# gergely-flamich/compression-without-quantization

Measured on AMD Instinct MI355X. Metric: latent blocks encoded/s at KL=16 bits, higher is better.
Workload: dtype f32

## Files before the change

### compression_without_quantization_amd/csrc/cwq_kernels.hip

```cpp
#include <hip/hip_runtime.h>

#include <type_traits>
#include <stdint.h>

#include "cwq_device.h"
#include "cwq_kernels.h"
#include "cwq_refill.h"
#include "cwq_tau_guess.h"

namespace cwq {

__global__ void __launch_bounds__(256) k_prep_dims(
    const float* __restrict__ t_scale, const float* __restrict__ p_loc,
    const float* __restrict__ p_scale, int64_t n, float nst, float sdiv, float rho,
    float* __restrict__ loc_s, float* __restrict__ scale_s, float* __restrict__ lognorm,
    float* __restrict__ out_sample, unsigned long long* __restrict__ keys, int64_t nb) {
  for (int64_t g = blockIdx.x * (int64_t)blockDim.x + threadIdx.x; g < nb;
       g += (int64_t)gridDim.x * blockDim.x)
    keys[g] = 0ull;
  for (int64_t i = blockIdx.x * (int64_t)blockDim.x + threadIdx.x; i < n;
       i += (int64_t)gridDim.x * blockDim.x) {
    float ls, ss;
    shard_consts(p_loc[i], p_scale[i], nst, sdiv, rho, ls, ss);
    loc_s[i] = ls;
    scale_s[i] = ss;
    lognorm[i] = lognorm_of(t_scale[i]);
    out_sample[i] = 0.0f;
  }
}

template <int DC, bool STEP0>
__device__ __forceinline__ float eval_row(const PhiloxStream& st, uint64_t kbase, int64_t d_rt,
                                          int align_rt, const float* __restrict__ loc_s,
                                          const float* __restrict__ scale_s,
                                          const float* __restrict__ mu,
                                          const float* __restrict__ sg,
                                          const float* __restrict__ lognorm,
                                          const float* __restrict__ best,
                                          const double* logtab) {
  return eval_row_f<DC>(st, kbase, d_rt, align_rt, logtab, [&](int64_t e, float zz) -> float {
    float s = scale_s[e] * zz;
    s = loc_s[e] + s;
    const float tv = STEP0 ? s : best[e] + s;
    return log_prob(tv, mu[e], sg[e], lognorm[e]);
  });
}

template <int DC, bool STEP0>
__global__ void __launch_bounds__(256) k_encode_eval(
    const float* __restrict__ t_loc, const float* __restrict__ t_scale,
    const float* __restrict__ loc_s, const float* __restrict__ scale_s,
    const float* __restrict__ lognorm, const float* __restrict__ best,
    const int64_t* __restrict__ block_off, int64_t ud, int64_t ntiles, int64_t tiles_per_block,
    int64_t cand_per_tile, int64_t n_cand, SeedSpec sd, int32_t step,
    unsigned long long* __restrict__ keys) {
  __shared__ double logtab[32];
  __shared__ unsigned long long wkey[4];
  fill_logtab(logtab);
  const uint32_t wv = wave_id();
  const uint32_t lane = threadIdx.x & 63u;

  for (int64_t tile = blockIdx.x; tile < ntiles; tile += gridDim.x) {
    const int64_t g = tile / tiles_per_block;
    const int64_t tt = tile - g * tiles_per_block;
    const BlockSpan sp = block_span(block_off, ud, g);
    const int64_t n0 = tt * cand_per_tile;
    const int64_t n1 = (n0 + cand_per_tile < n_cand) ? n0 + cand_per_tile : n_cand;
    const PhiloxStream st =
        generate_key(step_seed(sd.of(g), step), 42);
    const int align = (int)(((uint64_t)(n0 + wv) * (uint64_t)sp.d) & 3u);

    uint64_t bestk = 0;
    for (int64_t n = n0 + 4 * (int64_t)lane + wv; n < n1; n += 256) {
      const float v = eval_row<DC, STEP0>(st, (uint64_t)n * (uint64_t)sp.d, sp.d, align,
                                          loc_s + sp.off, scale_s + sp.off, t_loc + sp.off,
                                          t_scale + sp.off, lognorm + sp.off,
                                          STEP0 ? nullptr : best + sp.off, logtab);
      const uint64_t k = argmax_key(v, (uint32_t)n);
      bestk = k > bestk ? k : bestk;
    }
    bestk = wave_max_u64(bestk);
    if (lane == 0) wkey[wv] = bestk;
    __syncthreads();
    if (threadIdx.x == 0) {
      uint64_t m = wkey[0];
      for (int i = 1; i < 4; ++i) m = wkey[i] > m ? wkey[i] : m;
      if (m) atomicMax(&keys[g], (unsigned long long)m);
    }
    __syncthreads();
  }
}

constexpr float kPruneC1 = 0x1p-14f;
#ifndef CWQ_PRUNE_MIN_WAVES
#define CWQ_PRUNE_MIN_WAVES 6
#endif
#ifndef CWQ_XCD_BALANCE
#define CWQ_XCD_BALANCE 1
#endif
#ifndef CWQ_TAU_SHARE_MASK
#define CWQ_TAU_SHARE_MASK 7u
#endif
#ifndef CWQ_CSR_TAU_SHARE_MASK
#define CWQ_CSR_TAU_SHARE_MASK 15u
#endif
#ifndef CWQ_SURVIVOR_CAP
#define CWQ_SURVIVOR_CAP 1024
#endif
#ifndef CWQ_LINKED_VISIT
#define CWQ_LINKED_VISIT 1
#endif
#ifndef CWQ_FOLD_ROUND0
#define CWQ_FOLD_ROUND0 1
#endif
#ifndef CWQ_BORROW_REFILL
#define CWQ_BORROW_REFILL 1
#endif
#ifndef CWQ_POOL_RANGE_SKIP
#define CWQ_POOL_RANGE_SKIP 1
#endif
#ifndef CWQ_PARK_COMPLETE
#define CWQ_PARK_COMPLETE 1
#endif
#ifndef CWQ_PARK_MIN_ROWS
#define CWQ_PARK_MIN_ROWS 8192
#endif
#ifndef CWQ_PARK_MIN_D
#define CWQ_PARK_MIN_D 16
#endif
#if CWQ_PARK_COMPLETE && !(CWQ_LINKED_VISIT && CWQ_BORROW_REFILL)
#error "CWQ_PARK_COMPLETE needs CWQ_LINKED_VISIT and CWQ_BORROW_REFILL"
#endif

template <bool STEP0>
__device__ __forceinline__ float cand_diff(float z, float ls, float ss, float mu, float bb) {
  const float s = shard_sample(ls, ss, z);
  const float tv = STEP0 ? s : bb + s;
  return tv - mu;
}
__device__ __forceinline__ float lp_from_z(float z, float cc) {
  const float u = -0.5f * (z * z);
  return u - cc;
}


struct VisitRec {
  float4 sa, sb;
  uint32_t add[2];
  int bk;
  int next;
};
static_assert(sizeof(VisitRec) == 48, "VisitRec: 48 bytes");

template <int D, bool STEP0>
__device__ __forceinline__ float score_rows_wave(
    const PhiloxStream& st, const uint32_t* rows, uint32_t cnt, const float* __restrict__ loc_s,
    const float* __restrict__ scale_s, const float* __restrict__ mu,
    const float* __restrict__ sg, const float* __restrict__ lognorm,
    const float* __restrict__ best, const double* logtab, float* buf, uint32_t lane) {
  constexpr uint32_t G = D / 4;
  const uint32_t r = lane / G, u = lane - r * G;
  if (r < cnt) {
    const F4 z = normal4_dev(st, (uint64_t)rows[r] * G + u, logtab);
#pragma unroll
    for (int t = 0; t < 4; ++t) {
      const uint32_t j = 4u * u + (uint32_t)t;
      const float zz = t == 0 ? z.a : (t == 1 ? z.b : (t == 2 ? z.c : z.d));
      float v = scale_s[j] * zz;
      v = loc_s[j] + v;
      const float tv = STEP0 ? v : best[j] + v;
      buf[r * D + j] = log_prob(tv, mu[j], sg[j], lognorm[j]);
    }
  }
  __builtin_amdgcn_fence(__ATOMIC_SEQ_CST, "wavefront");
  __builtin_amdgcn_wave_barrier();
  float acc = 0.0f;
  const uint32_t fr = lane >> 3;
  if (fr < cnt)
    for (uint32_t e = lane & 7u; e < (uint32_t)D; e += 8u) acc = acc + buf[fr * D + e];
  __builtin_amdgcn_fence(__ATOMIC_SEQ_CST, "wavefront");
  __builtin_amdgcn_wave_barrier();
  float p[8];
#pragma unroll
  for (int l = 0; l < 8; ++l) p[l] = __shfl(acc, (int)((lane & ~7u) + (uint32_t)l), 64);
  return eigen_fold8(p, 0.0f);
}

#ifdef CWQ_TILE_TIMES
constexpr int kTileTimes = 1 << 18;
__device__ unsigned long long g_tile_t0[kTileTimes], g_tile_t1[kTileTimes];
__device__ unsigned int g_tile_wg[kTileTimes];
#endif
#ifdef CWQ_PRUNE_STATS
__device__ unsigned long long g_prune_stats[72];
constexpr int kDbgBlocks = 1 << 20;
__device__ unsigned long long g_dbg_best[kDbgBlocks];
__device__ int g_seed_tau;
#endif

struct TauGuessWaveDims {
  float w, b2;
  int d;
  __device__ __forceinline__ int count() const { return d; }
  template <class F>
  __device__ __forceinline__ cwq::TauGuessSums sum(F f) const {
    cwq::TauGuessSums o = f(w, b2);
#pragma unroll
    for (int sh = 32; sh >= 1; sh >>= 1) {
      o.k += __shfl_xor(o.k, sh, 64);
      o.k1 += __shfl_xor(o.k1, sh, 64);
      o.k2 += __shfl_xor(o.k2, sh, 64);
    }
    return o;
  }
};
__device__ __forceinline__ uint64_t sgpr_pair_uniform(uint64_t v) {
  const uint32_t lo = (uint32_t)__builtin_amdgcn_readfirstlane((int)(uint32_t)v);
  const uint32_t hi = (uint32_t)__builtin_amdgcn_readfirstlane((int)(uint32_t)(v >> 32));
  return ((uint64_t)hi << 32) | lo;
}
constexpr float kTauForceRetry = -2.0f;
__device__ __forceinline__ float tau_guess_of(float qm, float As, float Pq) {
  if (qm == kTauForceRetry) return 3.402823466e+38f;
  if (!(qm >= 0.0f)) return -__builtin_inff();
  const float tg = cwq::screen_row_lower(-qm, cwq::kScreenC2, As, Pq);
  return tg == tg ? tg : -__builtin_inff();
}

template <int D, bool STEP0, bool INTER, bool PARK>
__global__ void __launch_bounds__(256, CWQ_PRUNE_MIN_WAVES) k_encode_prune(
    const float* __restrict__ t_loc, const float* __restrict__ t_scale,
    const float* __restrict__ loc_s, const float* __restrict__ scale_s,
    const float* __restrict__ lognorm, const float* __restrict__ best, int64_t ntiles,
    int64_t tiles_per_block, int64_t cand_per_tile, int64_t n_cand, SeedSpec sd, int32_t step,
    int allow_screen, unsigned long long* __restrict__ keys, int64_t tail_from, int tail_div,
    uint32_t* __restrict__ tq) {
  static_assert(D % 8 == 0 && D >= 8 && D <= 64, "pruned path: D % 8 == 0, D <= 64");
  static_assert(!PARK || CWQ_PARK_COMPLETE, "PARK instances exist in CWQ_PARK_COMPLETE builds only");
  constexpr int G = D / 4;
  constexpr int NF = STEP0 ? 6 : 7;
  constexpr int RW = (64 / G) < 8 ? (64 / G) : 8;
  __shared__ double logtab[32];
  __shared__ float4 cst[G * NF];
  constexpr int NREC = CWQ_FOLD_ROUND0 ? 4 : 1;
  constexpr int RPW = G + (PARK ? 1 : 0);
  __shared__ VisitRec vrec[NREC * RPW];
  __shared__ uint32_t w0g_cell[4];
  __shared__ int2 meta[G];
  __shared__ float rowbuf[4][RW * D];
  __shared__ float dscore[D];
  __shared__ float dA[D];
  __shared__ float dC[D];
  __shared__ float gscore[G];
  __shared__ int gpos[G];
  __shared__ float lowc;
  __shared__ float scr_a, scr_pq;
  __shared__ float tau_cell;
  __shared__ float tau_seed_cell;
  __shared__ float qm_cell;
  __shared__ uint32_t sq_cnt;
  __shared__ uint32_t sq_n[CWQ_SURVIVOR_CAP];
  __shared__ float sq_ub[CWQ_SURVIVOR_CAP];
  __shared__ unsigned long long wkey[4];
  __shared__ uint32_t s_next;
#ifdef CWQ_PRUNE_STATS
  __shared__ uint32_t s_ps[72];
  for (int i = threadIdx.x; i < 72; i += blockDim.x) s_ps[i] = 0u;
#endif
  fill_logtab(logtab);
  const uint32_t wv = wave_id();
  const uint32_t lane = threadIdx.x & 63u;

  constexpr bool inter = INTER;
  const int64_t nbt = INTER ? ntiles / tiles_per_block : 0;
  auto next_tile = [&](int64_t cur) -> int64_t {
    if (tq == nullptr) return cur + gridDim.x;
    __syncthreads();
    if (threadIdx.x == 0) s_next = gridDim.x + atomicAdd(tq, 1u);
    __syncthreads();
    return (int64_t)s_next;
  };
  for (int64_t tile = blockIdx.x; tile < ntiles; tile = next_tile(tile)) {
    uint32_t tid = threadIdx.x;
    asm volatile("" : "+v"(tid));
#ifdef CWQ_TILE_TIMES
    if (tid == 0 && tile < kTileTimes) {
      g_tile_t0[tile] = __builtin_amdgcn_s_memrealtime();
      const uint32_t xcc = (uint32_t)__builtin_amdgcn_s_getreg((20) | (0 << 6) | ((4 - 1) << 11));
      g_tile_wg[tile] = (xcc << 24) | (blockIdx.x & 0xffffffu);
    }
#endif
    int64_t tord = tile;
    const int64_t treg = inter ? nbt * tail_from : 0;
    if (inter && CWQ_XCD_BALANCE && tq == nullptr && tile < treg && (treg & 7) == 0 &&
        (gridDim.x & 7u) == 0)
      tord = (tile & 7) * (treg >> 3) + (tile >> 3);
    const int64_t g = inter ? tord % nbt : tile / tiles_per_block;
    const int64_t tt = inter ? tord / nbt : tile - g * tiles_per_block;
    const int64_t off = g * D;
    int64_t n0, csz;
    if (tt < tail_from) {
      n0 = tt * cand_per_tile;
      csz = cand_per_tile;
    } else {
      csz = cand_per_tile / tail_div;
      n0 = tail_from * cand_per_tile + (tt - tail_from) * csz;
    }
    const int64_t n1 = (n0 + csz < n_cand) ? n0 + csz : n_cand;
    if (n0 >= n1) continue;
    const PhiloxStream st =
        generate_key(step_seed(sd.of(g), step), 42);

    if (tid < D) {
      const int j = tid;
      const float ls = loc_s[off + j], ss = scale_s[off + j], mu = t_loc[off + j];
      const float rs = 1.0f / t_scale[off + j];
      const float m = (STEP0 ? ls : best[off + j] + ls) - mu;
      float e = 0.5f * (ss * ss + m * m) * (rs * rs);
      dscore[j] = (e == e) ? e : -1.0f;
    }
    __syncthreads();
    if (tid < G) {
      const int q = tid;
      gscore[q] = ((dscore[4 * q] + dscore[4 * q + 1]) + dscore[4 * q + 2]) + dscore[4 * q + 3];
    }
    __syncthreads();
    if (tid < G) {
      const int q = tid;
      const float sq = gscore[q];
      int r = 0;
      for (int q2 = 0; q2 < G; ++q2) {
        const float s2 = gscore[q2];
        r += (s2 > sq || (s2 == sq && q2 < q)) ? 1 : 0;
      }
      gpos[q] = r;
      meta[r].x = q;
#pragma unroll
      for (int w = 0; w < NREC; ++w) {
        const uint32_t wg = (uint32_t)(n0 + (int64_t)w * ((n1 - n0 + 3) / 4)) * (uint32_t)G;
        const uint64_t add =
            CWQ_FOLD_ROUND0 ? cwq::philox_round0_addend(wg + (uint32_t)q) : (uint64_t)q;
        VisitRec& v = vrec[w * RPW + r];
        v.add[0] = (uint32_t)add;
        v.add[1] = (uint32_t)(add >> 32);
        v.next = (r + 1 < G || PARK) ? (w * RPW + r + 1) * (int)sizeof(VisitRec) : 0;
      }
    }
    if (PARK && tid >= 64 && tid < 64 + NREC) {
      VisitRec& v = vrec[(tid - 64) * RPW + G];
      v.sa = float4{0.f, 0.f, 0.f, 0.f};
      v.sb = float4{0.f, 0.f, 0.f, 0.f};
      v.add[0] = 0u;
      v.add[1] = 0u;
      v.bk = (int)f2u(__builtin_inff());
      v.next = (int)((tid - 64) * RPW + G) * (int)sizeof(VisitRec);
    }
    __syncthreads();
    int den_ok = 1, scr_ok = 1;
    if (tid < D) {
      const int j = tid, k = gpos[j >> 2], w = j & 3;
      float fj[7];
      const float sgj = t_scale[off + j];
      fj[0] = loc_s[off + j];
      fj[1] = scale_s[off + j];
      fj[2] = t_loc[off + j];
      fj[3] = sgj;
      fj[4] = lognorm[off + j];
      fj[5] = 1.0f / sgj;
      fj[6] = STEP0 ? 0.0f : best[off + j];
      float* c = reinterpret_cast<float*>(cst);
#pragma unroll
      for (int f = 0; f < NF; ++f) c[(k * NF + f) * 4 + w] = fj[f];
      den_ok = markstein_ok_den(sgj) ? 1 : 0;
      const ScreenDim o = screen_dim<STEP0>(fj[0], fj[1], fj[2], sgj, fj[4], fj[6]);
#pragma unroll
      for (int c = 0; c < NREC; ++c) {
        float* sc = reinterpret_cast<float*>(&vrec[c * RPW + k]);
        sc[w] = o.sa;
        sc[4 + w] = o.sb;
      }
      dA[j] = o.A;
      dC[j] = o.C;
      scr_ok = o.ok ? 1 : 0;
    }
    const bool fastdiv = __syncthreads_and(den_ok) != 0;
    const bool scr_all = __syncthreads_and(scr_ok) != 0;
    const bool screen = (allow_screen & 1) && scr_all;
    if (wv == 1u) {
      const int gmode = (allow_screen >> 1) & 3;
      float qm = cwq::kTauNoGuess;
      if (screen && gmode == 1) {
        float w = 0.0f, b2 = 0.0f;
        if (lane < (uint32_t)D) {
          const float* sc = reinterpret_cast<const float*>(&vrec[lane >> 2]);
          const float al = sc[lane & 3u] * (float)(1.0 / cwq::kSqrt2Ln2);
          const float be = sc[4u + (lane & 3u)];
          w = al * al;
          b2 = be * be;
        }
        qm = cwq::tau_guess_q(TauGuessWaveDims{w, b2, D}, n1 - n0, cwq::kTauGuessM);
      } else if (screen && gmode == 2) {
        qm = kTauForceRetry;
      }
      if (lane == 0) qm_cell = qm;
    }
    if (tid <= G + 1) {
      const int kb = tid;
      const float* c = reinterpret_cast<const float*>(cst);
      double rf = 0.0, kk = 0.0, asum = 0.0, msum = 0.0, kall = 0.0, cvis = 0.0, a2 = 0.0,
             amax = 0.0;
#pragma unroll 1
      for (int p = 0; p < D; ++p) {
        const double mj = -(double)c[((p >> 2) * NF + 4) * 4 + (p & 3)];
        const double aj = __builtin_fabs(mj);
        asum += aj;
        msum += mj;
        kall += aj + mj;
        if (p >= 4 * kb) {
          rf += mj + 0x1p-17 * aj;
        } else {
          kk += aj + mj;
          if (screen) cvis += (double)dC[(meta[p >> 2].x << 2) + (p & 3)];
        }
        if (screen && kb == G + 1) {
          const double av = (double)dA[p];
          a2 += av * av;
          amax = av > amax ? av : amax;
        }
      }
      const double marg = 0x1p-20 * (__builtin_fabs(rf) + asum) + 0x1p-126;
      const double sl = 0x1p-14 * (__builtin_fabs(msum) + asum + kall) + 0x1p-126;
      if (kb <= G) {
        const float bk = screen ? round_up_f32(msum + cvis * (1.0 + 0x1p-20) + sl)
                                : round_up_f32(rf + 0x1p-14 * kk + marg);
        if (kb >= 1) {
          meta[kb - 1].y = (int)f2u(bk);
#pragma unroll
          for (int c = 0; c < NREC; ++c) vrec[c * RPW + kb - 1].bk = (int)f2u(bk);
        }
        if (kb == G) lowc = round_up_f32(0x1p-14 * kk + marg);
      } else if (screen) {
        scr_a = screen_as(msum, sl, a2);
        scr_pq = screen_pq(amax, D);
      }
      if (kb == 0) {
        float t0 = -__builtin_inff();
        if (inter) {
          const unsigned long long kv =
              __hip_atomic_load(&keys[g], __ATOMIC_RELAXED, __HIP_MEMORY_SCOPE_AGENT);
          if ((uint32_t)(kv >> 32) > kArgmaxClampOrd) t0 = unord_f32((uint32_t)(kv >> 32));
        }
#ifdef CWQ_PRUNE_STATS
        if (g_seed_tau && g < kDbgBlocks && (g_dbg_best[g] >> 32) > kArgmaxClampOrd)
          t0 = unord_f32((uint32_t)(g_dbg_best[g] >> 32));
#endif
        tau_cell = t0;
        tau_seed_cell = t0;
        sq_cnt = 0u;
      }
    }
    __syncthreads();
    const float lc = lowc;
#ifdef CWQ_PRUNE_STATS
    const float tau_seed = tau_cell;
#endif
    const float sA = scr_a, sPq = scr_pq;

    const int64_t per_wave = (n1 - n0 + 3) / 4;
    const int64_t w0 = n0 + (int64_t)wv * per_wave;
    const int64_t w1 = (w0 + per_wave < n1) ? w0 + per_wave : n1;
    const uint32_t w0g =
        (uint32_t)__builtin_amdgcn_readfirstlane((int)((uint32_t)w0 * (uint32_t)G));
    if (lane == 0) w0g_cell[wv] = w0g;
    const uint32_t wrows = w1 > w0 ? (uint32_t)(w1 - w0) : 0u;
    const uint32_t ng_end =
        (uint32_t)__builtin_amdgcn_readfirstlane((int)(wrows * (uint32_t)G));
    const uint32_t ng_stat = (uint32_t)__builtin_amdgcn_readfirstlane(
        (int)(cwq::refill_static_rows(wrows) * (uint32_t)G));
    const uint32_t ng_pool0 = (uint32_t)__builtin_amdgcn_readfirstlane(
        (int)(cwq::refill_pool_start(cwq::refill_static_rows(wrows)) * (uint32_t)G));
    const uint32_t ng_first =
        (CWQ_BORROW_REFILL && ng_stat != 0u) ? ng_stat - 64u * (uint32_t)G : 0u;
    const uint32_t kbase = CWQ_FOLD_ROUND0 ? wv * (uint32_t)(RPW * sizeof(VisitRec)) : 0u;
#ifndef CWQ_TAU_FROM_KEYS
#define CWQ_TAU_FROM_KEYS 1
#endif
    float tau = (INTER && CWQ_TAU_FROM_KEYS) ? tau_cell : -__builtin_inff();
#ifdef CWQ_PRUNE_STATS
    tau = tau_seed;
    if (tid == 0 && qm_cell >= 0.0f) atomicAdd(&g_prune_stats[50], 1ull);
#endif
    tau = max_f32_quiet(tau, tau_guess_of(qm_cell, sA, sPq));
    uint64_t bestk = 0;

    const PhiloxLo lok = philox_lo_key(st);
    auto pass = [&](auto screen_tag) {
      constexpr bool SCREEN = decltype(screen_tag)::value;
      constexpr uint32_t KS = SCREEN ? (uint32_t)sizeof(VisitRec) : 1u;
      constexpr bool LINKED = SCREEN && CWQ_LINKED_VISIT;
      constexpr bool PARKED = SCREEN && PARK && CWQ_PARK_COMPLETE;
      uint32_t ng = ng_first + lane * (uint32_t)G;
      uint32_t wnext_g = ng_pool0;
      uint64_t left;
      asm volatile("s_cmp_eq_u32 %1, 0\n\ts_cselect_b64 %0, -1, 0" : "=s"(left) : "s"(ng_stat) : "scc");
      const uint32_t kb = SCREEN ? kbase : 0u;
      uint32_t kp = kb;
      float s = 0.0f;
      uint32_t iter = 0;
      uint32_t w0g_x = 0u;
      if constexpr (!SCREEN || !CWQ_FOLD_ROUND0) w0g_x = w0g;
      bool active = ng < ng_end;
      uint64_t m_act = __builtin_amdgcn_ballot_w64(active);
      while (m_act != 0ull) {
        int2 mt;
        float4 sa, sb;
        uint32_t kp_next = 0;
        uint64_t p0;
#ifdef CWQ_PRUNE_STATS
        const uint32_t kp_was = kp;
#endif
        if constexpr (SCREEN) {
          const char* rp = reinterpret_cast<const char*>(vrec) + kp;
          sa = *reinterpret_cast<const float4*>(rp);
          sb = *reinterpret_cast<const float4*>(rp + 16);
          typedef int v4i __attribute__((ext_vector_type(4)));
          v4i lk = *reinterpret_cast<const v4i*>(rp + 32);
          if constexpr (CWQ_FOLD_ROUND0) asm volatile("" : "+v"(lk));
          mt = int2{lk.x, lk.z};
          kp_next = (uint32_t)lk.w;
          if constexpr (CWQ_FOLD_ROUND0) {
            p0 = cwq::philox_round0_product(
                ng, (uint64_t)(uint32_t)lk.x | ((uint64_t)(uint32_t)lk.y << 32));
          } else {
            p0 = (uint64_t)kPhiloxM0 * ((ng + (uint32_t)mt.x) + w0g_x);
          }
        } else {
          mt = meta[kp];
          p0 = (uint64_t)kPhiloxM0 * ((ng + (uint32_t)mt.x) + w0g_x);
        }
        uint32_t pk0 = st.k0, pk1 = st.k1;
        asm volatile("" : "+s"(pk0), "+s"(pk1));
        const U4 x = philox10_lo_p0(p0, lok, pk0, pk1);
        float z0, z1, z2, z3;
        float upper;
        if constexpr (SCREEN) {
          box_muller_screen(x.x, x.y, z0, z1);
          box_muller_screen(x.z, x.w, z2, z3);
          const float a0 = __builtin_fmaf(sa.x, z0, sb.x);
          const float a1 = __builtin_fmaf(sa.y, z1, sb.y);
          const float a2 = __builtin_fmaf(sa.z, z2, sb.z);
          const float a3 = __builtin_fmaf(sa.w, z3, sb.w);
          s = __builtin_fmaf(-a0, a0, s);
          s = __builtin_fmaf(-a1, a1, s);
          s = __builtin_fmaf(-a2, a2, s);
          s = __builtin_fmaf(-a3, a3, s);
          upper = screen_row_upper(s, kScreenC1, u2f((uint32_t)mt.y));
        } else {
          box_muller_dev(x.x, x.y, logtab, z0, z1);
          box_muller_dev(x.z, x.w, logtab, z2, z3);
          const float4* cq = cst + kp * NF;
          const float4 ls = cq[0], ss = cq[1], mu = cq[2], sg = cq[3], cc = cq[4], ry = cq[5];
          const float4 bb = STEP0 ? float4{0.f, 0.f, 0.f, 0.f} : cq[6];
          const float d0 = cand_diff<STEP0>(z0, ls.x, ss.x, mu.x, bb.x);
          const float d1 = cand_diff<STEP0>(z1, ls.y, ss.y, mu.y, bb.y);
          const float d2 = cand_diff<STEP0>(z2, ls.z, ss.z, mu.z, bb.z);
          const float d3 = cand_diff<STEP0>(z3, ls.w, ss.w, mu.w, bb.w);
          float y0 = div_rn_markstein(d0, sg.x, ry.x);
          float y1 = div_rn_markstein(d1, sg.y, ry.y);
          float y2 = div_rn_markstein(d2, sg.z, ry.z);
          float y3 = div_rn_markstein(d3, sg.w, ry.w);
          const bool ok = fastdiv & markstein_ok4(d0, d1, d2, d3);
          if (__builtin_expect(__ballot(!ok) != 0ull, 0)) {
            if (!ok) {
              y0 = d0 / sg.x;
              y1 = d1 / sg.y;
              y2 = d2 / sg.z;
              y3 = d3 / sg.w;
            }
          }
          s = s + lp_from_z(y0, cc.x);
          s = s + lp_from_z(y1, cc.y);
          s = s + lp_from_z(y2, cc.z);
          s = s + lp_from_z(y3, cc.w);
          upper = (s + __builtin_fabsf(s) * kPruneC1) + u2f((uint32_t)mt.y);
        }
        if constexpr (LINKED)
          kp = kp_next;
        else
          kp += KS;
        const bool complete =
            PARKED ? false : (LINKED ? (kp == 0u) : (kp == kb + KS * (uint32_t)G));
        const bool below = upper < tau;
        const bool reach = SCREEN ? !below : (upper >= tau);
#ifdef CWQ_PRUNE_STATS
        const bool complete_st =
            PARKED ? (kp == kb + KS * (uint32_t)G && kp_was != kb + KS * (uint32_t)G) : complete;
        const bool prune = !complete_st && below;
        const uint32_t k = (LINKED && complete_st) ? (uint32_t)G : (kp - kb) / KS;
#endif
        const bool done = complete || below || !active;
        const uint64_t m_cpl = __builtin_amdgcn_ballot_w64(complete);
        const uint64_t m_below = __builtin_amdgcn_fcmpf(upper, tau, 4 );
        uint64_t m = m_cpl | m_below | (__builtin_amdgcn_read_exec() & ~m_act);
        uint64_t m_keep =
            m_cpl & m_act &
            (SCREEN ? ~m_below : (uint64_t)__builtin_amdgcn_fcmpf(upper, tau, 3 ));
        asm volatile("" : "+s"(m), "+s"(m_keep));
        auto keep_rows = [&](const uint64_t mk) {
          const bool keep = CWQ_BORROW_REFILL ? ((mk >> lane) & 1ull) != 0ull
                                              : (complete && active && reach);
          float lower;
          if constexpr (SCREEN)
            lower = screen_row_lower(s, kScreenC2, sA, sPq);
          else
            lower = (s - __builtin_fabsf(s) * kPruneC1) - lc;
          if constexpr (PARKED) {
            uint32_t kf = (uint32_t)G - 1u;
            asm volatile("" : "+v"(kf));
            upper = screen_row_upper(s, kScreenC1, u2f((uint32_t)meta[kf].y));
          }
          tau = tau_raise_wave(tau, keep, lower);
          if (__builtin_expect(keep && upper >= tau, 0)) {
            uint32_t ngc = ng;
            asm volatile("" : "+v"(ngc));
            const uint32_t n =
                (*const_cast<const volatile uint32_t*>(&w0g_cell[wv]) + ngc) / (uint32_t)G;
#ifdef CWQ_PRUNE_STATS
            atomicAdd(&s_ps[66], 1u);
#endif
            const uint32_t slot = atomicAdd(&sq_cnt, 1u);
            if (slot < CWQ_SURVIVOR_CAP) {
              sq_n[slot] = (uint32_t)n;
              sq_ub[slot] = upper;
            } else {
#ifdef CWQ_PRUNE_STATS
              atomicAdd(&g_prune_stats[69], 1ull);
#endif
              const float v = eval_row<D, STEP0>(st, (uint64_t)n * D, D, 0, loc_s + off,
                                                 scale_s + off, t_loc + off, t_scale + off,
                                                 lognorm + off, STEP0 ? nullptr : best + off, logtab);
              const uint64_t kv = argmax_key(v, (uint32_t)n);
              bestk = kv > bestk ? kv : bestk;
            }
          }
        };
        if constexpr (!PARKED) {
          if (__builtin_expect(m_keep != 0ull, 0)) keep_rows(m_keep);
        } else {
          if (((++iter) & CWQ_TAU_SHARE_MASK) == 0u) {
            tau = tau_share_wave(&tau_cell, tau);
            const uint64_t m_park =
                __builtin_amdgcn_uicmp(kp, kb + KS * (uint32_t)G, 32 ) & m_act & ~m_below;
            if (__builtin_expect(m_park != 0ull, 0)) keep_rows(m_park);
            m |= m_park;
          }
        }
#ifdef CWQ_PRUNE_STATS
        const bool act_l = ((m_act >> lane) & 1ull) != 0ull;
        if (act_l && (complete_st || prune)) atomicAdd(&s_ps[k], 1u);
        if (act_l && complete_st) atomicAdd(&s_ps[65], 1u);
#endif
        uint64_t m_pool;
        if constexpr (CWQ_BORROW_REFILL) {
          asm volatile(
              "s_mov_b64 exec, %[m]\n\t"
              "v_subrev_co_u32 %[ng], vcc, %[c], %[ng]\n\t"
              "v_mov_b32 %[kp], %[kb]\n\t"
              "v_mov_b32 %[s], 0\n\t"
              "s_mov_b64 exec, -1\n\t"
              "s_and_b64 %[mp], vcc, %[m]\n\t"
              "s_or_b64 %[left], %[left], %[mp]\n\t"
              "s_and_b64 %[mp], %[left], %[m]"
              : [ng] "+v"(ng), [kp] "+v"(kp), [s] "+v"(s), [mp] "=&s"(m_pool),
                [left] "+s"(left)
              : [m] "s"(m), [c] "n"(64 * G), [kb] "s"(kb)
              : "vcc", "scc");
          left = sgpr_pair_uniform(left);
          m_pool = sgpr_pair_uniform(m_pool);
        } else {
          if (done) {
            asm volatile("" : "+v"(ng));
            ng += 64u * (uint32_t)G;
            kp = kb;
            s = 0.0f;
          }
          m_pool = 0ull;
        }
        if (!PARKED && ((++iter) & CWQ_TAU_SHARE_MASK) == 0u) {
          tau = tau_share_wave(&tau_cell, tau);
        }
        if constexpr (CWQ_BORROW_REFILL) {
          if (m_pool != 0ull) {
#ifdef CWQ_PRUNE_STATS
            if (lane == 0) atomicAdd(&s_ps[70], 1u);
#endif
            const uint32_t rank = __builtin_amdgcn_mbcnt_hi(
                (uint32_t)(m_pool >> 32), __builtin_amdgcn_mbcnt_lo((uint32_t)m_pool, 0u));
            asm volatile(
                "s_mov_b64 exec, %[mp]\n\t"
                "v_mad_u32_u24 %[ng], %[rank], %[g], %[wn]\n\t"
                "s_mov_b64 exec, -1"
                : [ng] "+v"(ng)
                : [mp] "s"(m_pool), [rank] "v"(rank), [g] "n"(G), [wn] "s"(wnext_g));
            const uint32_t want = wnext_g + (uint32_t)__builtin_popcountll(m_pool) * (uint32_t)G;
            if (CWQ_POOL_RANGE_SKIP && want <= ng_end) {
              wnext_g = want;
              m_act |= m_pool;
            } else {
              wnext_g = want < ng_end ? want : ng_end;
              m_act = __builtin_amdgcn_uicmp(ng, ng_end, 36 );
            }
          }
        } else {
          m_pool = m & __builtin_amdgcn_uicmp(ng, ng_stat, 35 );
          if (m_pool != 0ull) {
#ifdef CWQ_PRUNE_STATS
            if (lane == 0) atomicAdd(&s_ps[70], 1u);
#endif
            const uint32_t rank = __builtin_amdgcn_mbcnt_hi(
                (uint32_t)(m_pool >> 32), __builtin_amdgcn_mbcnt_lo((uint32_t)m_pool, 0u));
            if (done && ng >= ng_stat) ng = wnext_g + rank * (uint32_t)G;
            wnext_g += (uint32_t)__builtin_popcountll(m_pool) * (uint32_t)G;
            wnext_g = wnext_g < ng_end ? wnext_g : ng_end;
            active = ng < ng_end;
            m_act = __builtin_amdgcn_ballot_w64(active);
          }
        }
#ifdef CWQ_PRUNE_STATS
        if (lane == 0) atomicAdd(&s_ps[71], 1u);
#endif
      }
    };
#ifdef CWQ_PRUNE_STATS
    if (screen && tid == 0) atomicAdd(&g_prune_stats[67], 1ull);
#endif
    float tau_final;
    if (screen) {
      for (;;) {
        pass(std::true_type{});
        tau_share_wave(&tau_cell, tau);
        __syncthreads();
        tau_final = tau_cell;
        const float tg = tau_guess_of(qm_cell, sA, sPq);
        const float seed = INTER ? tau_seed_cell : -__builtin_inff();
        const bool held = tau_final > tg || seed >= tg;
        if (__builtin_amdgcn_readfirstlane(held ? 1 : 0) != 0) break;
        __syncthreads();
        if (tid == 0) {
          tau_cell = seed;
          sq_cnt = 0u;
          qm_cell = cwq::kTauNoGuess;
#ifdef CWQ_PRUNE_STATS
          atomicAdd(&g_prune_stats[51], 1ull);
#endif
        }
        __syncthreads();
        tau = (INTER && CWQ_TAU_FROM_KEYS) ? seed : -__builtin_inff();
      }
    } else {
      pass(std::false_type{});
      tau_share_wave(&tau_cell, tau);
      __syncthreads();
      tau_final = tau_cell;
    }
    const uint32_t nsurv = sq_cnt < CWQ_SURVIVOR_CAP ? sq_cnt : CWQ_SURVIVOR_CAP;
    const uint32_t nsurv_u = (uint32_t)__builtin_amdgcn_readfirstlane((int)nsurv);
    const uint32_t sl = tid & 63u;
    for (uint32_t c0 = wv * 64u; c0 < nsurv_u; c0 += 256u) {
      const uint32_t i = c0 + sl;
      const bool q = i < nsurv_u && sq_ub[i] >= tau_final;
      const uint32_t nn = i < nsurv_u ? sq_n[i] : 0u;
      const uint64_t qm = __builtin_amdgcn_ballot_w64(q);
      if (qm == 0ull) continue;
#ifdef CWQ_PRUNE_STATS
      if (q) atomicAdd(&g_prune_stats[68], 1ull);
#endif
      const uint32_t qr = __builtin_amdgcn_mbcnt_hi((uint32_t)(qm >> 32),
                                                    __builtin_amdgcn_mbcnt_lo((uint32_t)qm, 0u));
      __builtin_amdgcn_fence(__ATOMIC_SEQ_CST, "wavefront");
      __builtin_amdgcn_wave_barrier();
      if (q) sq_n[c0 + qr] = nn;
      __builtin_amdgcn_fence(__ATOMIC_SEQ_CST, "wavefront");
      __builtin_amdgcn_wave_barrier();
      const uint32_t qn = (uint32_t)__builtin_popcountll(qm);
      for (uint32_t b = 0; b < qn; b += (uint32_t)RW) {
        const uint32_t cnt = qn - b < (uint32_t)RW ? qn - b : (uint32_t)RW;
        const float v = score_rows_wave<D, STEP0>(
            st, sq_n + c0 + b, cnt, loc_s + off, scale_s + off, t_loc + off, t_scale + off,
            lognorm + off, STEP0 ? nullptr : best + off, logtab, rowbuf[wv], sl);
        if ((sl & 7u) == 0u && (sl >> 3) < cnt) {
          const uint64_t kv = argmax_key(v, sq_n[c0 + b + (sl >> 3)]);
          bestk = kv > bestk ? kv : bestk;
        }
      }
    }

    bestk = wave_max_u64(bestk);
    if (lane == 0) wkey[wv] = bestk;
    __syncthreads();
    if (tid == 0) {
      uint64_t mk = wkey[0];
      for (int i = 1; i < 4; ++i) mk = wkey[i] > mk ? wkey[i] : mk;
      if (mk) atomicMax(&keys[g], (unsigned long long)mk);
#ifdef CWQ_PRUNE_STATS
      if (!g_seed_tau && g < kDbgBlocks) g_dbg_best[g] = mk;
#endif
#ifdef CWQ_TILE_TIMES
      if (tile < kTileTimes) g_tile_t1[tile] = __builtin_amdgcn_s_memrealtime();
#endif
    }
#ifdef CWQ_PRUNE_STATS
    if (tid < 72) {
      if (s_ps[tid]) atomicAdd(&g_prune_stats[tid], (unsigned long long)s_ps[tid]);
      s_ps[tid] = 0u;
    }
#endif
    __syncthreads();
  }
}

__device__ __forceinline__ double block_sum_d(double v, double* red) {
  red[threadIdx.x] = v;
  __syncthreads();
  for (int w = 128; w > 0; w >>= 1) {
    if ((int)threadIdx.x < w) red[threadIdx.x] += red[threadIdx.x + w];
    __syncthreads();
  }
  const double r = red[0];
  __syncthreads();
  return r;
}

__host__ __device__ __forceinline__ int64_t csr_cls_stride(int64_t d) { return (d + 6) / 4 + 1; }
constexpr int64_t kCsrSortUnits = 2048;

template <bool STEP0>
__global__ void __launch_bounds__(256) k_csr_prep(
    const float* __restrict__ t_loc, const float* __restrict__ t_scale,
    const float* __restrict__ loc_s, const float* __restrict__ scale_s,
    const float* __restrict__ lognorm, const float* __restrict__ best,
    const int64_t* __restrict__ block_off, int64_t ud, int64_t nb, float2* __restrict__ sab,
    float* __restrict__ cdim, float* __restrict__ bpre, uint32_t* __restrict__ ordu,
    float4* __restrict__ grp, uint32_t* __restrict__ gtau, float4* __restrict__ abp,
    int64_t lds_dims, int64_t coop_min_d) {
  __shared__ double red[5][4];
  __shared__ double wscan[4];
  __shared__ double ucs[256];
  __shared__ unsigned long long skey[kCsrSortUnits];
  const int tid = threadIdx.x;
  const int lane = tid & 63, wv = tid >> 6;
  const bool lead = blockIdx.y == 0;
  for (int64_t g = blockIdx.x; g < nb; g += gridDim.x) {
    const BlockSpan sp = block_span(block_off, ud, g);
    const int64_t off = sp.off, d = sp.d;
    ScreenSums u;
    float2* sabg = sab + off + 8 * g + 4;
    float* cg = cdim + off;
    if (lead && tid < 8) {
      if (tid < 4) sabg[tid - 4] = float2{0.f, 0.f};
      sabg[d + tid] = float2{0.f, 0.f};
    }
    for (int64_t j = tid; j < d; j += 256) {
      const ScreenDim o =
          screen_dim<STEP0>(loc_s[off + j], scale_s[off + j], t_loc[off + j], t_scale[off + j],
                            lognorm[off + j], STEP0 ? 0.0f : best[off + j]);
      sabg[j] = float2{o.sa, o.sb};
      cg[j] = o.C;
      u.add(o);
    }
    u.sm = wave_sum_f64(u.sm);
    u.sa = wave_sum_f64(u.sa);
    u.sk = wave_sum_f64(u.sk);
    u.s2 = wave_sum_f64(u.s2);
    u.mx = wave_max_f64(u.mx);
    if (lane == 0) {
      red[0][wv] = u.sm;
      red[1][wv] = u.sa;
      red[2][wv] = u.sk;
      red[3][wv] = u.s2;
      red[4][wv] = u.mx;
    }
    __threadfence_block();
    const bool all_ok = __syncthreads_and(u.ok) != 0;
    ScreenSums S;
    S.sm = ((red[0][0] + red[0][1]) + red[0][2]) + red[0][3];
    S.sa = ((red[1][0] + red[1][1]) + red[1][2]) + red[1][3];
    S.sk = ((red[2][0] + red[2][1]) + red[2][2]) + red[2][3];
    S.s2 = ((red[3][0] + red[3][1]) + red[3][2]) + red[3][3];
    S.mx = red[4][0];
    for (int w = 1; w < 4; ++w) S.mx = red[4][w] > S.mx ? red[4][w] : S.mx;
    const bool coop_blk = d >= coop_min_d;
    const ScreenBlock bc =
        screen_block_consts(S, d, coop_blk ? 16.0 + (double)d / 64.0 : (double)d);
    const double SM = S.sm, sl = bc.sl;
    const int64_t reg = off + 12 * g, cs = csr_cls_stride(d);
    const bool recs = abp != nullptr && d > lds_dims;
    auto sab_at = [&](int64_t j) {
      const unsigned long long v = __hip_atomic_load(
          reinterpret_cast<unsigned long long*>(sabg + j), __ATOMIC_RELAXED,
          __HIP_MEMORY_SCOPE_AGENT);
      return float2{u2f((uint32_t)v), u2f((uint32_t)(v >> 32))};
    };
    for (int c = (int)blockIdx.y; c < 4; c += (int)gridDim.y) {
      auto unit = [&](int64_t u, double& csum, double& gain) {
        csum = 0.0;
        gain = 0.0;
        for (int t = 0; t < 4; ++t) {
          const int64_t j = 4 * u - c + t;
          if (j >= 0 && j < d) {
            const float2 ab = sab_at(j);
            const float xc = u2f(__hip_atomic_load(reinterpret_cast<uint32_t*>(cg + j),
                                                   __ATOMIC_RELAXED, __HIP_MEMORY_SCOPE_AGENT));
            csum += (double)xc;
            gain += (double)ab.x * (double)ab.x * (0.5 / 0.6931471805599453) +
                    (double)ab.y * (double)ab.y - (double)xc;
          }
        }
      };
      auto key_of = [&](int64_t u) {
        double cu, gu;
        unit(u, cu, gu);
        const float gf = (float)(gu > 0.0 ? gu : 0.0);
        return ((unsigned long long)ord_f32(gf) << 32) | (0xffffffffull - (uint64_t)u);
      };
      const int64_t U = (d + c + 3) / 4;
      const bool sorted = all_ok && U <= kCsrSortUnits;
      const bool small = U <= 256;
      if (sorted && small) {
        unsigned long long key = 0ull;
        if (tid < U) {
          double cu, gu;
          unit(tid, cu, gu);
          ucs[tid] = cu;
          const float gf = (float)(gu > 0.0 ? gu : 0.0);
          key = ((unsigned long long)ord_f32(gf) << 32) | (0xffffffffull - (uint64_t)tid);
          skey[tid] = key;
        }
        __syncthreads();
        int r = 0;
        if (tid < U)
          for (int i = 0; i < (int)U; ++i) r += skey[i] > key ? 1 : 0;
        __syncthreads();
        if (tid < U) skey[r] = key;
        __syncthreads();
      } else if (sorted) {
        int64_t P = 1;
        while (P < U) P <<= 1;
        for (int64_t u = tid; u < P; u += 256) skey[u] = u < U ? key_of(u) : 0ull;
        __syncthreads();
        for (int64_t k = 2; k <= P; k <<= 1) {
          for (int64_t jj = k >> 1; jj > 0; jj >>= 1) {
            for (int64_t i = tid; i < P; i += 256) {
              const int64_t l = i ^ jj;
              if (l > i) {
                const unsigned long long x = skey[i], y = skey[l];
                const bool desc = (i & k) == 0;
                if (desc ? (x < y) : (x > y)) {
                  skey[i] = y;
                  skey[l] = x;
                }
              }
            }
            __syncthreads();
          }
        }
      }
      double carry = 0.0;
      for (int64_t base = 0; base <= U; base += 256) {
        const int64_t k = base + tid;
        int64_t u = k;
        if (sorted && k < U) u = (int64_t)(0xffffffffull - (skey[k] & 0xffffffffull));
        double cu = 0.0, gu;
        if (all_ok && k < U) {
          if (sorted && small)
            cu = ucs[u];
          else
            unit(u, cu, gu);
        }
        if (recs && k <= U) {
          float e[8];
          for (int t = 0; t < 4; ++t) {
            const int64_t j = 4 * u - c + t;
            float2 ab = float2{0.f, 0.f};
            if (k < U && j >= 0 && j < d) ab = sab_at(j);
            e[2 * t] = ab.x;
            e[2 * t + 1] = ab.y;
          }
          float4* rr = abp + 2 * (csr_rec_base(off) + c * cs + k);
          rr[0] = float4{e[0], e[1], e[2], e[3]};
          rr[1] = float4{e[4], e[5], e[6], e[7]};
        }
        double v = cu;
#pragma unroll
        for (int o = 1; o < 64; o <<= 1) {
          const double t = __shfl_up(v, (unsigned)o, 64);
          if (lane >= o) v += t;
        }
        if (lane == 63) wscan[wv] = v;
        __syncthreads();
        double pre = 0.0;
        for (int w = 0; w < wv; ++w) pre += wscan[w];
        const double total = ((wscan[0] + wscan[1]) + wscan[2]) + wscan[3];
        const double excl = carry + (pre + v) - cu;
        if (k <= U) {
          bpre[reg + c * cs + k] = round_up_f32(SM + excl * (1.0 + 0x1p-20) + sl);
          ordu[reg + c * cs + k] = (uint32_t)(k < U ? u : U);
        }
        carry += total;
        __syncthreads();
      }
    }
    if (lead && tid == 0) {
      grp[g] = (all_ok && bc.finite && d > 0) ? float4{bc.c1, bc.c2, bc.as, bc.pq}
                                              : float4{0.f, 0.f, 0.f, 0.f};
      gtau[g * CWQ_CSR_GTAU_STRIDE] = ord_f32(-__builtin_inff());
    }
    __syncthreads();
  }
}

constexpr int kRowChunk = 248;

template <bool STEP0>
__device__ __forceinline__ float exact_row_wave(
    const PhiloxStream& st, uint64_t kbase, int64_t d, const float* __restrict__ loc_s,
    const float* __restrict__ scale_s, const float* __restrict__ mu,
    const float* __restrict__ sg, const float* __restrict__ lognorm,
    const float* __restrict__ best, const double* logtab, float* buf, uint32_t lane) {
  const int64_t vec = d & ~(int64_t)7;
  float acc = 0.0f;
  for (int64_t j0 = 0; j0 < d; j0 += kRowChunk) {
    const int64_t cnt = (d - j0) < kRowChunk ? d - j0 : kRowChunk;
    const uint64_t k0 = kbase + (uint64_t)j0;
    const uint64_t blk = (k0 >> 2) + lane;
// ... 2534 lines not shown
```

### compression_without_quantization_amd/csrc/cwq_refill.h

```cpp
#pragma once
#include <stdint.h>

#if defined(__HIPCC__)
#define CWQ_REFILL_HD __host__ __device__ __forceinline__
#else
#define CWQ_REFILL_HD inline
#endif

namespace cwq {

constexpr uint32_t kRefillLanes = 64;
constexpr uint32_t kRefillMinRows = 128;

CWQ_REFILL_HD uint32_t refill_static_rows(uint32_t R) {
  if (R < kRefillMinRows) return 0u;
  const uint32_t s = (uint32_t)(((uint64_t)R * 7u) >> 3);
  return s & ~(kRefillLanes - 1u);
}

CWQ_REFILL_HD uint32_t refill_pool_start(uint32_t S) { return S < kRefillLanes ? kRefillLanes : S; }

}
```

Before: 3.916 million.

## Unroll parked screening loop with compile-time share/look scheduling in fast path

For the PARK screen pass, the while loop body becomes a lambda that runs unrolled U times (default 8) while the wave is fully active and enough pool rows remain. Tau-share and park-look checks are decided at compile time per unrolled copy, and the inactive-lane masking and range checks are dropped in this fast path. A normal single-iteration loop handles the tail. This targets per-iteration scalar overhead and branching, at the cost of code size and register pressure and more complex iteration-count bookkeeping.

```diff
diff --git a/compression_without_quantization_amd/csrc/cwq_kernels.hip b/compression_without_quantization_amd/csrc/cwq_kernels.hip
--- a/compression_without_quantization_amd/csrc/cwq_kernels.hip
+++ b/compression_without_quantization_amd/csrc/cwq_kernels.hip
@@ -130,6 +130,15 @@
 #endif
 #if CWQ_PARK_COMPLETE && !(CWQ_LINKED_VISIT && CWQ_BORROW_REFILL)
 #error "CWQ_PARK_COMPLETE needs CWQ_LINKED_VISIT and CWQ_BORROW_REFILL"
+#endif
+#ifndef CWQ_SHARE_UNROLL
+#define CWQ_SHARE_UNROLL 8
+#endif
+#ifndef CWQ_PARK_LOOK_MASK
+#define CWQ_PARK_LOOK_MASK CWQ_TAU_SHARE_MASK
+#endif
+#if CWQ_SHARE_UNROLL != 1 && CWQ_SHARE_UNROLL != 2 && CWQ_SHARE_UNROLL != 4 && CWQ_SHARE_UNROLL != 8
+#error "CWQ_SHARE_UNROLL is 1, 2, 4 or 8"
 #endif
 
 template <bool STEP0>
@@ -225,6 +234,11 @@
   if (!(qm >= 0.0f)) return -__builtin_inff();
   const float tg = cwq::screen_row_lower(-qm, cwq::kScreenC2, As, Pq);
   return tg == tg ? tg : -__builtin_inff();
+}
+
+template <class F, uint32_t... I>
+__device__ __forceinline__ void unroll_each(F& f, std::integer_sequence<uint32_t, I...>) {
+  (f(std::integral_constant<uint32_t, I>{}, std::integral_constant<uint32_t, (uint32_t)sizeof...(I)>{}), ...);
 }
 
 template <int D, bool STEP0, bool INTER, bool PARK>
@@ -511,7 +525,20 @@
       if constexpr (!SCREEN || !CWQ_FOLD_ROUND0) w0g_x = w0g;
       bool active = ng < ng_end;
       uint64_t m_act = __builtin_amdgcn_ballot_w64(active);
-      while (m_act != 0ull) {
+      constexpr uint32_t U = PARKED ? (uint32_t)CWQ_SHARE_UNROLL : 1u;
+      constexpr uint32_t LOOK_MASK = PARKED ? (uint32_t)(CWQ_PARK_LOOK_MASK) : 0u;
+      static_assert(LOOK_MASK <= CWQ_TAU_SHARE_MASK, "a look at least as often as a share");
+      auto body = [&](auto copy_tag, auto unroll_tag) {
+        constexpr uint32_t C = decltype(copy_tag)::value;
+        constexpr uint32_t UU = decltype(unroll_tag)::value;
+        constexpr bool FAST = UU > 1u;
+        constexpr bool COUNTS = cwq::unroll_counts<CWQ_TAU_SHARE_MASK, UU>() ||
+                                cwq::unroll_counts<LOOK_MASK, UU>();
+        if constexpr (COUNTS && C + 1u == UU) iter += UU;
+        const bool share_due = cwq::unroll_due<CWQ_TAU_SHARE_MASK, UU, C>(iter);
+#ifdef CWQ_PRUNE_STATS
+        if (lane == 0) atomicAdd(&s_ps[71], 1u);
+#endif
         int2 mt;
         float4 sa, sb;
         uint32_t kp_next = 0;
@@ -601,11 +628,17 @@
         const bool done = complete || below || !active;
         const uint64_t m_cpl = __builtin_amdgcn_ballot_w64(complete);
         const uint64_t m_below = __builtin_amdgcn_fcmpf(upper, tau, 4 );
-        uint64_t m = m_cpl | m_below | (__builtin_amdgcn_read_exec() & ~m_act);
+        uint64_t m = m_cpl | m_below;
+        if constexpr (!FAST) m |= __builtin_amdgcn_read_exec() & ~m_act;
         uint64_t m_keep =
-            m_cpl & m_act &
+            m_cpl & (FAST ? ~0ull : m_act) &
             (SCREEN ? ~m_below : (uint64_t)__builtin_amdgcn_fcmpf(upper, tau, 3 ));
-        asm volatile("" : "+s"(m), "+s"(m_keep));
+        constexpr bool LOOK_HERE =
+            PARKED && (C + 1u == UU || (LOOK_MASK + 1u <= UU && ((C + 1u) & LOOK_MASK) == 0u));
+        if constexpr (!PARKED)
+          asm volatile("" : "+s"(m), "+s"(m_keep));
+        else if constexpr (!FAST || LOOK_HERE)
+          asm volatile("" : "+s"(m));
         auto keep_rows = [&](const uint64_t mk) {
           const bool keep = CWQ_BORROW_REFILL ? ((mk >> lane) & 1ull) != 0ull
                                               : (complete && active && reach);
@@ -647,10 +680,10 @@
         if constexpr (!PARKED) {
           if (__builtin_expect(m_keep != 0ull, 0)) keep_rows(m_keep);
         } else {
-          if (((++iter) & CWQ_TAU_SHARE_MASK) == 0u) {
-            tau = tau_share_wave(&tau_cell, tau);
-            const uint64_t m_park =
-                __builtin_amdgcn_uicmp(kp, kb + KS * (uint32_t)G, 32 ) & m_act & ~m_below;
+          if (share_due) tau = tau_share_wave(&tau_cell, tau);
+          if (cwq::unroll_due<LOOK_MASK, UU, C>(iter)) {
+            const uint64_t m_park = __builtin_amdgcn_uicmp(kp, kb + KS * (uint32_t)G, 32 ) &
+                                    (FAST ? ~0ull : m_act) & ~m_below;
             if (__builtin_expect(m_park != 0ull, 0)) keep_rows(m_park);
             m |= m_park;
           }
@@ -686,11 +719,11 @@
           }
           m_pool = 0ull;
         }
-        if (!PARKED && ((++iter) & CWQ_TAU_SHARE_MASK) == 0u) {
+        if (!PARKED && share_due) {
           tau = tau_share_wave(&tau_cell, tau);
         }
         if constexpr (CWQ_BORROW_REFILL) {
-          if (m_pool != 0ull) {
+          if (FAST ? __builtin_expect(m_pool != 0ull, 0) : (m_pool != 0ull)) {
 #ifdef CWQ_PRUNE_STATS
             if (lane == 0) atomicAdd(&s_ps[70], 1u);
 #endif
@@ -703,7 +736,9 @@
                 : [ng] "+v"(ng)
                 : [mp] "s"(m_pool), [rank] "v"(rank), [g] "n"(G), [wn] "s"(wnext_g));
             const uint32_t want = wnext_g + (uint32_t)__builtin_popcountll(m_pool) * (uint32_t)G;
-            if (CWQ_POOL_RANGE_SKIP && want <= ng_end) {
+            if constexpr (FAST) {
+              wnext_g = want;
+            } else if (CWQ_POOL_RANGE_SKIP && want <= ng_end) {
               wnext_g = want;
               m_act |= m_pool;
             } else {
@@ -726,10 +761,14 @@
             m_act = __builtin_amdgcn_ballot_w64(active);
           }
         }
-#ifdef CWQ_PRUNE_STATS
-        if (lane == 0) atomicAdd(&s_ps[71], 1u);
-#endif
-      }
+      };
+      constexpr std::integral_constant<uint32_t, 0u> c0{};
+      constexpr std::integral_constant<uint32_t, 1u> u1{};
+      if constexpr (U > 1u) {
+        while (m_act == ~0ull && wnext_g + cwq::unroll_trip_rows(U) * (uint32_t)G <= ng_end)
+          unroll_each(body, std::make_integer_sequence<uint32_t, U>{});
+      }
+      while (m_act != 0ull) body(c0, u1);
     };
 #ifdef CWQ_PRUNE_STATS
     if (screen && tid == 0) atomicAdd(&g_prune_stats[67], 1ull);
diff --git a/compression_without_quantization_amd/csrc/cwq_refill.h b/compression_without_quantization_amd/csrc/cwq_refill.h
--- a/compression_without_quantization_amd/csrc/cwq_refill.h
+++ b/compression_without_quantization_amd/csrc/cwq_refill.h
@@ -20,4 +20,19 @@
 
 CWQ_REFILL_HD uint32_t refill_pool_start(uint32_t S) { return S < kRefillLanes ? kRefillLanes : S; }
 
+template <uint32_t M, uint32_t U, uint32_t C>
+CWQ_REFILL_HD bool unroll_due(uint32_t iters) {
+  static_assert((M & (M + 1u)) == 0u && (U & (U - 1u)) == 0u && U >= 1u && C < U,
+                "unroll_due: M + 1 and U are powers of two, C < U");
+  if constexpr (M + 1u <= U)
+    return ((C + 1u) & M) == 0u;
+  else if constexpr (C + 1u != U)
+    return false;
+  else
+    return (iters & M) == 0u;
 }
+template <uint32_t M, uint32_t U>
+constexpr bool unroll_counts() { return M + 1u > U; }
+constexpr uint32_t unroll_trip_rows(uint32_t U) { return U * kRefillLanes; }
+
+}
```

Measured after the change: 3.974 million (median of 6 runs). 1.01x the previous value.
